# shuaigroup/Renormalizer

Measured on AMD Instinct MI355X. Metric: TDVP-PS sweep site-updates/sec at (Nsite=50, Dbond=256, dphys=2/16), higher is better.
Workload: dtype c128

## Files before the change

include/mpsengine.h:

```cpp
#ifndef MPSENGINE_H
#define MPSENGINE_H

#include <stddef.h>
#include <stdint.h>

#ifdef __cplusplus
extern "C" {
#endif

typedef struct mpse_ctx mpse_ctx;

enum {
  MPSE_OK = 0,
  MPSE_ERR_OOM = 1,
  MPSE_ERR_SHAPE = 2,
  MPSE_ERR_NOCONV = 3,
  MPSE_ERR_HIP = 4,
  MPSE_ERR_ARG = 5
};

enum { MPSE_F64 = 0, MPSE_C128 = 1 };
enum { MPSE_DOMAIN_L = 0, MPSE_DOMAIN_R = 1 };


// ... 56 lines not shown
  int conj_a, conj_b;
  mpse_index m_a, k_a;
  mpse_index k_b, n_b;
  mpse_index m_c, n_c;
  int64_t batch;
  int64_t sb_a, sb_b, sb_c;
  double alpha_re, alpha_im;
  double beta_re, beta_im;
  int skip_zero_tiles;
} mpse_gemm_desc;

int mpse_gemm(mpse_ctx* ctx, const mpse_gemm_desc* desc, const void* A, const void* B, void* C);

int mpse_gemm_path_stats(mpse_ctx* ctx, int64_t* counts, int n);

int mpse_transpose_inner(mpse_ctx* ctx, int dtype, void* out, const void* in,
                         int64_t d0, int64_t d1, int64_t d2, int conj);


typedef struct {
  int64_t Dl_bra, Dl_ket;
  int64_t Dr_bra, Dr_ket;
  int64_t d0, d1;
  int64_t danc;
  int64_t wl, wm, wr;
  int64_t env_unit;
  int64_t danc1;
} mpse_dims;

int mpse_env_update(mpse_ctx* ctx, int dtype, int domain, const mpse_dims* dims,
// ... 159 lines not shown
```

renormalizer_amd/csrc/mpse_cholqr.hip:

```cpp
#include <type_traits>

#include "mpse_device.h"
#include "mpse_internal.h"

typedef double v4d __attribute__((ext_vector_type(4)));

namespace {

struct CqBlk {
  long long ws_off;
  long long part_off;
  long long t_off;
  long long row_off, col_off;
  int mm, nn, P, T;
  int nchunk, rpc;
  int koff, pad;
};

__device__ __forceinline__ v4d mfma(double a, double b, v4d c) {
  return __builtin_amdgcn_mfma_f64_16x16x4f64(a, b, c, 0, 0, 0);
}
__device__ __forceinline__ double readlane_d(double v, int l) {
  const int lo = __builtin_amdgcn_readlane(__double2loint(v), l);
  const int hi = __builtin_amdgcn_readlane(__double2hiint(v), l);
// ... 775 lines not shown
        st2<CPLX>(Vt, (koff + c) * ncol + cols[r], vr, -vi);
      }
    } else {
      const long long u = t - tq;
      const int c = (int)(u % nn), i = (int)(u / nn);
      double vr = 0.0, vi = 0.0;
      if (i <= c) ld2<CPLX>(Rt, (long long)tile_index(i >> 4, c >> 4, B.P) * 256 + (i & 15) * 16 + (c & 15), vr, vi);
      if (!herm)
        st2<CPLX>(Vt, (koff + i) * ncol + cols[c], vr, vi);
      else
        st2<CPLX>(U, rows[c] * K + koff + i, vr, -vi);
    }
  }
}

template <bool CPLX>
int cholqr_run(mpse_ctx* ctx, double* ws, const QrBlk* blks, int nblk, const long long* drows, const long long* dcols,
               int herm, void* U, void* Vt, long long K, long long ncol, bool* ok) {
  MPSE_TRY(qr_words(ctx));
  int* gflag = ctx->qr_optimistic ? ctx->qr_words_dev : nullptr;
  constexpr size_t es = CPLX ? 16 : 8;
  std::vector<CqBlk> cb(nblk);
  long long part_tot = 0, t_tot = 0;
  int max_gram = 1, max_T = 1, max_nrb = 1, max_P = 1;
  long long max_sc = 1;
  long long groups = 0;
  for (int b = 0; b < nblk; ++b) {
    const int P2 = ((blks[b].nn + 15) / 16 + 1) / 2;
    groups += P2 * (P2 + 1) / 2;
  }
  for (int b = 0; b < nblk; ++b) {
    CqBlk& c = cb[b];
    c.ws_off = blks[b].ws_off;
    c.mm = blks[b].mm;
    c.nn = blks[b].nn;
    c.P = (c.nn + 15) / 16;
    c.T = c.P * (c.P + 1) / 2;
    c.row_off = blks[b].row_off;
    c.col_off = blks[b].col_off;
    c.koff = blks[b].prm_off;
    c.pad = 0;
    int want = (int)((8LL * ctx->n_cu + groups - 1) / groups);
    if (want < 1) want = 1;
    if (want > 64) want = 64;
    int rpc = (c.mm + want - 1) / want;
    if (rpc < 32) rpc = 32;
    rpc = (rpc + 3) & ~3;
    c.rpc = rpc;
    c.nchunk = (c.mm + rpc - 1) / rpc;
    c.part_off = part_tot;
    c.t_off = t_tot;
    part_tot += (long long)((c.nchunk + 3) / 4) * c.T * 256;
    t_tot += c.T;
    {
      const int P2 = (c.P + 1) / 2, T2 = P2 * (P2 + 1) / 2;
      max_gram = std::max(max_gram, ((c.nchunk + 3) / 4) * T2);
    }
    max_T = std::max(max_T, c.T);
    max_P = std::max(max_P, c.P);
    max_nrb = std::max(max_nrb, (c.mm + 15) / 16);
    max_sc = std::max<long long>(max_sc, (long long)c.mm * c.nn + (long long)c.nn * c.nn);
  }
  const size_t db = (size_t(nblk) * sizeof(CqBlk) + 15) & ~size_t(15);
  const size_t pb = size_t(part_tot) * es, tb = size_t(t_tot) * 256 * es, ib = size_t(t_tot) * 2 * sizeof(double);
  const size_t sb = ((2 * size_t(nblk) + 1) * sizeof(int) + 15) & ~size_t(15);
  TmpBuf M(ctx);
  MPSE_TRY(M.alloc(db + pb + 6 * tb + ib + sb + 16));
  char* base = static_cast<char*>(M.p);
  MPSE_TRY(stage_h2d(ctx, base, cb.data(), size_t(nblk) * sizeof(CqBlk)));
  const CqBlk* dblk = reinterpret_cast<const CqBlk*>(base);
  double* part = reinterpret_cast<double*>(base + db);
  double* G = reinterpret_cast<double*>(base + db + pb);
  double* Rb[5];
  for (int i = 0; i < 5; ++i) Rb[i] = reinterpret_cast<double*>(base + db + pb + (1 + i) * tb);
  double* tinfo = reinterpret_cast<double*>(base + db + pb + 6 * tb);
  int* status = reinterpret_cast<int*>(base + db + pb + 6 * tb + ib);
  const int* done = status + 1 + nblk;
  double* dstat = reinterpret_cast<double*>(base + db + pb + 6 * tb + ib + sb);
  static const double theta = [] {
    const char* e = getenv("MPSE_CHOLQR_THETA");
    return e ? atof(e) : 1e-12;
  }();
  static const double tau = [] {
    const char* e = getenv("MPSE_CHOLQR_TAU");
    return e ? atof(e) : 0.1;
// ... 45 lines not shown
  static const int min_rows = [] {
    const char* e = getenv("MPSE_CHOLQR_MINROWS");
    return e ? atoi(e) : 256;
  }();
  if (mode == 0 || nblk <= 0) return false;
  int max_mm = 0, max_nn = 0;
  for (int b = 0; b < nblk; ++b) {
    if (blks[b].mm < blks[b].nn || blks[b].k != blks[b].nn || blks[b].nn > 256) return false;
    max_mm = std::max(max_mm, blks[b].mm);
    max_nn = std::max(max_nn, blks[b].nn);
  }
  if (mode >= 2) return true;
  return max_mm >= min_rows && max_nn >= 96;
}

int cholqr_blocks(mpse_ctx* ctx, bool cplx, double* ws, const QrBlk* blks, int nblk, const long long* drows,
                  const long long* dcols, int herm, void* U, void* Vt, long long K, long long ncol, bool* ok) {
  *ok = false;
  if (cplx) return cholqr_run<true>(ctx, ws, blks, nblk, drows, dcols, herm, U, Vt, K, ncol, ok);
  return cholqr_run<false>(ctx, ws, blks, nblk, drows, dcols, herm, U, Vt, K, ncol, ok);
}
```

renormalizer_amd/csrc/mpse_gemm.hip:

```cpp
#include <cstdlib>

#include "mpse_device.h"
#include "mpse_internal.h"
#include "mpse_plans.h"

typedef double v4d __attribute__((ext_vector_type(4)));

static unsigned long long* gemm_trace_ptr(const mpse_ctx* ctx) {
  static const bool f0_only = [] {
    const char* e = getenv("MPSE_GEMM_TRACE_ONLY");
    return e && e[0] == 'f';
  }();
  return (ctx->prof_on && !f0_only) ? ctx->gemm_trace : nullptr;
}

namespace {

struct IdxMap {
  long long s_hi, s_lo;
  int ext, lo;
};

constexpr int GMAX_GRP = 8, GMAX_SEG = 4, GMAX_MIX = 8;
struct GMix {
// ... 865 lines not shown
      dre = dim = 0.0;
#pragma unroll
      for (int w = 0; w < NT / 64; ++w) {
        dre += s_dot[2 * w];
        dim += s_dot[2 * w + 1];
      }
      if (tid == 0) {
        const long long slot = (long long)bs * ntile + (long long)tm * g.tiles_n + tn;
        g.dot_part[2 * slot] = dre;
        g.dot_part[2 * slot + 1] = dim;
      }
    }
  }
}

__device__ __forceinline__ void bitonic_desc(unsigned* key, int tid, int n) {
  for (int size = 2; size <= n; size <<= 1)
    for (int stride = size >> 1; stride > 0; stride >>= 1) {
      if (tid < (n >> 1)) {
        const int lo = 2 * tid - (tid & (stride - 1)), hi = lo + stride;
        const bool desc = (lo & size) == 0;
        const unsigned a = key[lo], b = key[hi];
        if ((a < b) == desc) {
          key[lo] = b;
          key[hi] = a;
        }
      }
      __syncthreads();
    }
}
__device__ __forceinline__ int pow2_at_least(int x) {
  int n = 2;
  while (n < x) n <<= 1;
  return n;
}
__global__ __launch_bounds__(1024) void k_tile_order(const unsigned long long* __restrict__ amask,
                                                       const unsigned long long* __restrict__ bmask, int nkw, int nkt,
                                                       int tiles_m, int tiles_n, int by_die, int* __restrict__ perm,
                                                       const int* __restrict__ skip, const GemmGroups gg,
                                                       unsigned char* __restrict__ flags_out, int flags_pitch,
                                                       int om_M, int om_N) {
  if (skip && *skip) return;
  __shared__ unsigned key[2048], ckey[2048];
  __shared__ int colw[2048];
  __shared__ unsigned char die_of[2048], dead[2048];
  const int ntile = tiles_m * tiles_n, tid = threadIdx.x;
  const bool part = by_die && tiles_n % 8 == 0 && tiles_n <= 2048;
  for (int c = tid; c < 2048; c += 1024) colw[c] = 0;
  __syncthreads();
  for (int i = tid; i < 2048; i += 1024) {
    unsigned cnt = 0;
    dead[i] = 0;
    if (i < ntile) {
      const int tm = i / tiles_n, tn = i - tm * tiles_n;
      if (gg.ngrp > 0) {
        const int grp = tm / gg.tiles_m_grp, tml = tm - grp * gg.tiles_m_grp;
        const GGrp& G = gg.g[grp];
        const bool off = gg.omask && !mpse_plan::out_tile_live(gg.omask, gg.om_pitch, gg.om_d, om_N, om_M, tm, tn);
        dead[i] = off ? 1 : 0;
        for (int q = 0; q < G.nseg; ++q)
          for (int l = 0; l < gg.nkt_seg; ++l) {
            unsigned v = off ? 0 : 1;
            if (G.seg[q].am) v &= G.seg[q].am[(long long)tml * gg.am_pitch + l];
            if (G.seg[q].bm) v &= G.seg[q].bm[(long long)tn * gg.bm_pitch + l];
            cnt += v;
            if (flags_out) flags_out[(long long)i * flags_pitch + q * gg.nkt_seg + l] = (unsigned char)v;
          }
        if (flags_out)
          for (int l = G.nseg * gg.nkt_seg; l < flags_pitch; ++l) flags_out[(long long)i * flags_pitch + l] = 0;
      } else {
        for (int w = 0; w < nkw; ++w) {
          unsigned long long x = 0x0101010101010101ull;
          if (amask) x &= amask[(long long)tm * nkw + w];
          if (bmask) x &= bmask[(long long)tn * nkw + w];
          const int valid = nkt - 8 * w;
          if (valid < 8) x &= (1ull << (8 * valid)) - 1ull;
          cnt += __popcll(x);
        }
      }
      if (part) atomicAdd(&colw[tn], (int)cnt);
    }
    key[i] = cnt;
  }
  __syncthreads();
  if (part) {
    for (int c = tid; c < 2048; c += 1024) ckey[c] = c < tiles_n ? ((unsigned)colw[c] << 11) | (unsigned)(2047 - c) : 0u;
    __syncthreads();
    bitonic_desc(ckey, tid, pow2_at_least(tiles_n));
    for (int r = tid; r < tiles_n; r += 1024) {
      const int c = 2047 - (int)(ckey[r] & 2047u), r16 = r & 15;
      die_of[c] = (unsigned char)(r16 < 8 ? r16 : 15 - r16);
    }
    __syncthreads();
  }
  for (int i = tid; i < 2048; i += 1024) {
    unsigned k = 0;
    if (i < ntile) {
      const unsigned die = part ? die_of[i % tiles_n] : 0u;
      k = (die << 28) | (key[i] << 16) | (unsigned)(0xFFFF - i);
    }
    key[i] = k;
  }
  __syncthreads();
  bitonic_desc(key, tid, pow2_at_least(ntile));
  const int per_die = ntile / 8;
  for (int i = tid; i < ntile; i += 1024) {
    const int s = part ? (7 - (i & 7)) * per_die + (i >> 3) : i;
    const int t = 0xFFFF - (int)(key[s] & 0xFFFFu);
    perm[i] = dead[t] ? ~t : t;
  }
}

template <bool CC>
__global__ __launch_bounds__(256) void k_splitk_reduce(const GemmArgs g, int batch) {
  constexpr int EC = CC ? 2 : 1;
  if (g.skip && *g.skip) return;
  const long long mn = (long long)g.M * g.N;
  const int rows = g.M * batch;
  double dre = 0.0, dim = 0.0;
  for (int row = blockIdx.y; row < rows; row += gridDim.y) {
    const int b = row / g.M;
    const int i = row - b * g.M;
    const double* wrow = g.ws + ((long long)b * g.ksplit * mn + (long long)i * g.N) * EC;
    double* crow = g.C + ((long long)b * g.sbC + idx_off(g.mC, i)) * EC;
    for (int j = blockIdx.x * 256 + threadIdx.x; j < g.N; j += gridDim.x * 256) {
// ... 406 lines not shown
      const OccOperand oa = occ_operand(ka, g.mA, g.kA, g.a_kfast, ma), ob = occ_operand(kb, g.nB, g.kB, g.b_kfast, mb);
      const dim3 og((p.nkt + 3) / 4, oa.tiles > ob.tiles ? oa.tiles : ob.tiles, (unsigned)(2 * d->batch));
      hipLaunchKernelGGL(k_tile_occ, og, dim3(256), 0, ctx->stream, oa, ob, g.K, g.nkw, (int)d->batch, g.skip);
    }
    g.amask = static_cast<const unsigned long long*>(ma.mask);
    g.bmask = static_cast<const unsigned long long*>(mb.mask);
  }

  if (p.order) {
    SolveScope* const keep = sc && sc->keeps_env_masks && ma.stable && mb.stable ? sc : nullptr;
    int* pp = nullptr;
    bool sort = false;
    MPSE_TRY(perm_source(ctx, keep, {g.amask, g.bmask, g.tiles_m, g.tiles_n, p.nkt, nullptr},
                         size_t(g.tiles_m) * g.tiles_n * sizeof(int), PERM, &pp, &sort));
    if (sort)
      hipLaunchKernelGGL(k_tile_order, dim3(1), dim3(1024), 0, ctx->stream, g.amask, g.bmask, g.nkw, p.nkt, g.tiles_m,
                         g.tiles_n, 1, pp, g.skip, GemmGroups(), (unsigned char*)nullptr, 0, 0, 0);
    g.perm = pp;
  }

  count_paths(ctx->gemm_paths, p, d->batch > 1);
  const bool reduce = g.ksplit > 1 && !p.leave_slices;
  launch_gemm(ctx, g, p.nwg, ca, cb, p.fast, p.wide, false, reduce ? dim3((unsigned)p.rgx, (unsigned)p.rgy) : dim3(0),
              (int)d->batch);
  if (prof_this) prof_end(ctx, rec);
  MPSE_HIP(ctx, hipGetLastError());
  return MPSE_OK;
}

int occ_mask_get(mpse_ctx* ctx, SolveScope* sc, const void* ptr, int dtype, mpse_index r, mpse_index k,
                 TmpBuf& tmp, const unsigned char** flags, int* pitch, bool* stable) {
  IdxMap rm, km;
// ... 130 lines not shown
  const bool prof_this = prof_begin(ctx, variant, mnk * ((ca && cb) ? 8.0 : 4.0),
                                    grouped_bytes(d, double(g.M), double(g.N), double(g.K), ca),
                                    &rec);
  g.kt_counter = prof_this && ctx->prof_ktiles ? ctx->prof_ktiles + variant : nullptr;

  TmpBuf PERM(ctx);
  if (p.order) {
    const size_t perm_bytes = (size_t(ntile) * sizeof(int) + 7) & ~size_t(7), flag_pitch = size_t(g.nkw) * 8;
    int* pp = nullptr;
    bool sort = false;
    MPSE_TRY(perm_source(ctx, sc && sc->keeps_env_masks && d.masks_stable ? sc : nullptr,
                         {gg.g[0].seg[0].am, gg.g[0].seg[0].bm, g.tiles_m, g.tiles_n,
                          nkt_max + 1000 * d.ngrp + (out_mask ? 1000000 : 0), nullptr},
                         perm_bytes + size_t(ntile) * flag_pitch, PERM, &pp, &sort));
    if (sort)
      hipLaunchKernelGGL(k_tile_order, dim3(1), dim3(1024), 0, ctx->stream, (const unsigned long long*)nullptr,
                         (const unsigned long long*)nullptr, 0, nkt_max, g.tiles_m, g.tiles_n, d.split2 ? 0 : 1, pp,
                         g.skip, gg, reinterpret_cast<unsigned char*>(pp) + perm_bytes, (int)flag_pitch, g.M, g.N);
    g.perm = pp;
    g.gg.flags = reinterpret_cast<const unsigned long long*>(reinterpret_cast<const char*>(pp) + perm_bytes);
  }

  count_paths(ctx->gemm_paths, d);
  ctx->gemm_paths[mpse_ctx::GP_GROUPED_OUTMASK] += out_mask;
  const bool om_wide = out_mask && d.split2 && ca && !p.wide && g.N % BN == 0;
  gg.dot4 = om_wide ? 1 : 0;
  launch_gemm(ctx, g, p.nwg, ca, cb, true, p.wide || om_wide, true);
  if (prof_this) prof_end(ctx, rec);
  MPSE_HIP(ctx, hipGetLastError());
  return MPSE_OK;
}

extern "C" int mpse_gemm(mpse_ctx* ctx, const mpse_gemm_desc* d, const void* A, const void* B, void* C) {
  if (ctx && d && MPSE_RECORDING(ctx)) {
    const mpse_gemm_desc dc = *d;
    ctx->defer_ops[ctx->defer_recording].push_back([ctx, dc, A, B, C] { return mpse_gemm(ctx, &dc, A, B, C); });
    return MPSE_OK;
  }
  return gemm_impl(ctx, d, A, B, C, d ? (d->skip_zero_tiles & 3) : 0, nullptr, nullptr);
}

extern "C" int mpse_gemm_path_stats(mpse_ctx* ctx, int64_t* counts, int n) {
  if (!ctx || n < 0 || (n > 0 && !counts)) return MPSE_ERR_ARG;
  for (int i = 0; i < n && i < mpse_ctx::GP_COUNT; ++i) counts[i] = ctx->gemm_paths[i];
  return MPSE_OK;
}

int gemm_call(mpse_ctx* ctx, int dta, int dtb, int conja, int conjb, mpse_index ma, mpse_index ka, mpse_index kb,
              mpse_index nb, mpse_index mc, mpse_index nc, int64_t batch, int64_t sba, int64_t sbb, int64_t sbc,
              const void* A, const void* B, void* C, double alpha, double beta, int skip_zero, SolveScope* sc,
              ProductReq* rq) {
  mpse_gemm_desc d;
  d.dtype_a = dta;
  d.dtype_b = dtb;
  d.conj_a = conja;
  d.conj_b = conjb;
  d.m_a = ma;
  d.k_a = ka;
  d.k_b = kb;
// ... 34 lines not shown
```

renormalizer_amd/csrc/mpse_heff0.hip:

```cpp
#include "mpse_device.h"
#include "mpse_internal.h"

typedef double v4d __attribute__((ext_vector_type(4)));

namespace {

__device__ __forceinline__ v4d mfma(double a, double b, v4d c) {
  return __builtin_amdgcn_mfma_f64_16x16x4f64(a, b, c, 0, 0, 0);
}

constexpr int F0_TMAX = 16;
struct F0Term {
  int b, e, x, pad;
  double w;
};
struct F0Info {
  int unit;
  int nt;
  unsigned long long lts;
  unsigned long long frn;
  unsigned long long cts;
  unsigned bpack, epack;
  double w[4];
};
// ... 31 lines not shown
__device__ __forceinline__ void f0_flags(const double2* __restrict__ E, int D, int w, int nt, unsigned char* __restrict__ F,
                                         int rt, int b) {
  __shared__ int s_f[64];
  const int row = threadIdx.x >> 4, col = threadIdx.x & 15;
  if (threadIdx.x < 64) s_f[threadIdx.x] = 0;
  __syncthreads();
  const double2* base = E + ((long long)(16 * rt + row) * w + b) * D;
  for (int ct = 0; ct < nt; ++ct) {
    const double2 v = base[16 * ct + col];
    if (v.x != 0.0 || v.y != 0.0) s_f[ct] = 1;
  }
  __syncthreads();
  if ((int)threadIdx.x < nt) F[((long long)rt * w + b) * nt + threadIdx.x] = s_f[threadIdx.x] ? 1 : 0;
}

__global__ __launch_bounds__(256) void k_f0_prepare(const double2* __restrict__ L, const double2* __restrict__ R,
                                                     double2* __restrict__ rt, unsigned char* __restrict__ FL,
                                                     unsigned char* __restrict__ FR, int Dl, int Dr, int wl, int wr, int ntl,
                                                     int ntr, const int* __restrict__ skip) {
  if (skip && *skip) return;
  int blk = blockIdx.x;
  if (blk < ntl * wl) {
    f0_flags(L, Dl, wl, ntl, FL, blk / wl, blk % wl);
    return;
  }
  blk -= ntl * wl;
  if (blk < ntr * wr) {
    f0_flags(R, Dr, wr, ntr, FR, blk / wr, blk % wr);
    return;
  }
  blk -= ntr * wr;
  f0_transpose(rt, R, Dr, wr, blk, (int)gridDim.x - ntl * wl - ntr * wr);
}

__global__ __launch_bounds__(1024) void k_f0_valid(const unsigned char* __restrict__ FL, const unsigned char* __restrict__ FC,
                                                    const unsigned char* __restrict__ FR, const F0Term* __restrict__ terms,
                                                    const int* __restrict__ nterm, int wl, int wr, int d, int ntl, int ntr,
                                                    int nkc, int fc_pitch, unsigned long long* __restrict__ mask,
                                                    const int* __restrict__ skip) {
  if (skip && *skip) return;
  __shared__ unsigned long long s1[64], s2[64];
  const int nparts = wr * nkc, tid = threadIdx.x;
  if (tid < 64) s1[tid] = s2[tid] = 0;
  __syncthreads();
  for (int t = tid; t < ntl * nparts; t += 1024) {
    const int at = t / nparts, s = t - at * nparts, f = s / nkc, kc = s - f * nkc;
    bool any = false;
// ... 494 lines not shown
  const size_t o_fl = rt_bytes, o_fr = o_fl + fl_bytes, o_tm = o_fr + fr_bytes, o_nt = o_tm + tm_bytes, o_mk = o_nt + nt_bytes;
  const size_t o_od = o_mk + mk_bytes, tot_bytes = o_od + od_bytes;
  static const bool order_on = [] {
    const char* e = getenv("MPSE_F0_ORDER");
    return !(e && e[0] == '0');
  }();
  if (hit) {
    base = static_cast<char*>(fc.buf);
  } else {
    void* p = nullptr;
    if (fc.buf) mpse_free(ctx, fc.buf);
    fc = SolveScope::F0Cache();
    MPSE_TRY(mpse_malloc(ctx, tot_bytes, &p));
    fc.buf = p, fc.L = h->L, fc.R = h->R, fc.W = h->W0, fc.cmask = FC, fc.Dl = Dl, fc.Dr = Dr, fc.w = wr, fc.nsite = h->nsite;
    base = static_cast<char*>(p);
    {
      std::vector<char> up(tm_bytes + nt_bytes, 0);
      memcpy(up.data(), terms.data(), tm_bytes);
      memcpy(up.data() + tm_bytes, nterm.data(), size_t(wr) * sizeof(int));
      MPSE_TRY(stage_h2d(ctx, base + o_tm, up.data(), up.size()));
    }
    const long long nel = (long long)wr * Dr * Dr;
    int nb = (int)((nel + 255) / 256);
    if (nb > 2048) nb = 2048;
    hipLaunchKernelGGL(k_f0_prepare, dim3(ntl * wl + ntr * wr + nb), dim3(256), 0, ctx->stream,
                       static_cast<const double2*>(h->L), static_cast<const double2*>(h->R), reinterpret_cast<double2*>(base),
                       reinterpret_cast<unsigned char*>(base + o_fl), reinterpret_cast<unsigned char*>(base + o_fr), Dl, Dr, wl,
                       wr, ntl, ntr, skip);
    if (order_on)
      hipLaunchKernelGGL(k_f0_plan, dim3(1), dim3(1024), 0, ctx->stream, reinterpret_cast<const unsigned char*>(base + o_fl), FC,
                         reinterpret_cast<const unsigned char*>(base + o_fr), reinterpret_cast<const F0Term*>(base + o_tm),
                         reinterpret_cast<const int*>(base + o_nt), wl, wr, d, ntl, ntr, nkc, fc_pitch,
                         reinterpret_cast<unsigned long long*>(base + o_mk), ctx->n_cu > 0 ? ctx->n_cu : 256,
                         reinterpret_cast<F0Info*>(base + o_od), compact ? 1 : 0, skip);
    else
      hipLaunchKernelGGL(k_f0_valid, dim3(1), dim3(1024), 0, ctx->stream, reinterpret_cast<const unsigned char*>(base + o_fl), FC,
                         reinterpret_cast<const unsigned char*>(base + o_fr), reinterpret_cast<const F0Term*>(base + o_tm),
                         reinterpret_cast<const int*>(base + o_nt), wl, wr, d, ntl, ntr, nkc, fc_pitch,
                         reinterpret_cast<unsigned long long*>(base + o_mk), skip);
  }
  F0Args g{};
  g.L = static_cast<const double*>(h->L);
  g.Rt = reinterpret_cast<const double*>(base);
// ... 44 lines not shown
```

renormalizer_amd/csrc/mpse_internal.h:

```cpp
#pragma once
#include <hip/hip_runtime.h>

#include <cstdarg>
#include <cstdlib>
#include <cstdint>
#include <cstdio>
#include <cstring>
#include <functional>
#include <map>
#include <memory>
#include <mutex>
#include <string>
#include <unordered_map>
#include <vector>

#include "../../include/mpsengine.h"

struct mpse_ctx {
  int device = 0;
  hipStream_t stream = nullptr;
  int n_cu = 0;
  char err[512] = {0};
  char dev_name[128] = {0};

// ... 410 lines not shown
};
struct QrBlk {
  long long ws_off;
  long long q_off;
  int mm, nn, k;
  int prm_off;
  int nq = 0;
  long long row_off = 0, col_off = 0;
};
constexpr int HH_BATCH_MAX_ROWS = 4096;
constexpr unsigned long long GEMM_TRACE_CAP = 1ull << 21;
constexpr int GEMM_TRACE_WORDS = 10;
int hh_qr(mpse_ctx* ctx, bool cplx, double* ws, double* q, HhParam* prm, const QrBlk* blks_host, int nblk, bool form_q,
          const QrBlk* blks_dev = nullptr);
bool cholqr_eligible(const mpse_ctx* ctx, const QrBlk* blks, int nblk);
int cholqr_blocks(mpse_ctx* ctx, bool cplx, double* ws, const QrBlk* blks, int nblk, const long long* drows,
                  const long long* dcols, int herm, void* U, void* Vt, long long K, long long ncol, bool* ok);
int device_zero2(mpse_ctx* ctx, void* a, size_t abytes, void* b, size_t bbytes);
```

renormalizer_amd/csrc/mpse_qr.hip:

```cpp
#include "mpse_cx.h"
#include "mpse_device.h"
#include "mpse_internal.h"

namespace {

template <bool CPLX>
__global__ void k_gather_blocks(double* ws_base, const double* __restrict__ coef, long long ncol,
                                const long long* __restrict__ drows, const long long* __restrict__ dcols,
                                const QrBlk* __restrict__ blks, int herm) {
  const QrBlk B = blks[blockIdx.y];
  double* ws = ws_base + B.ws_off * Cx<CPLX>::E;
  const long long* rows = drows + B.row_off;
  const long long* cols = dcols + B.col_off;
  const int mm = B.mm, nn = B.nn;
  const long long total = (long long)mm * nn;
  const long long stride = (long long)gridDim.x * blockDim.x;
  for (long long t = (long long)blockIdx.x * blockDim.x + threadIdx.x; t < total; t += stride) {
    int r, c;
    if (!herm) {
      c = (int)(t % nn);
      r = (int)(t / nn);
      Cx<CPLX>::st(ws, r + (long long)c * mm, Cx<CPLX>::ld(coef, rows[r] * ncol + cols[c]));
    } else {
      r = (int)(t % mm);
// ... 83 lines not shown
  const int64_t nri = row_off[nblocks], nci = col_off[nblocks];
  int64_t max_el = 0, max_sc = 0;
  for (size_t i = 0; i < blks.size(); ++i) {
    blks[i].row_off = row_off[which[i]];
    blks[i].col_off = col_off[which[i]];
    max_el = std::max<int64_t>(max_el, (int64_t)blks[i].mm * blks[i].nn);
    max_sc = std::max<int64_t>(max_sc, (int64_t)blks[i].mm * blks[i].k + (int64_t)blks[i].k * blks[i].nn);
  }
  double qr_flops = 0.0, qr_bytes = 0.0;
  for (const QrBlk& B : blks) {
    const double m = B.mm, n = B.k;
    qr_flops += (CPLX ? 4.0 : 1.0) * (4.0 * m * n * n - 4.0 * n * n * n / 3.0);
    qr_bytes += double(es) * (2.0 * B.mm * B.nn + double(B.mm) * B.k);
  }
  ProfScope qprof(ctx, 5, qr_flops, qr_bytes);
  const size_t ib = size_t(nri + nci) * sizeof(int64_t), db = blks.size() * sizeof(QrBlk);
  static_assert(sizeof(QrBlk) % 8 == 0, "descriptors follow the 8-byte index lists");
  std::vector<char> host(ib + db);
  memcpy(host.data(), row_idx, size_t(nri) * sizeof(int64_t));
  memcpy(host.data() + size_t(nri) * sizeof(int64_t), col_idx, size_t(nci) * sizeof(int64_t));
  memcpy(host.data() + ib, blks.data(), db);
  TmpBuf IDX(ctx), WS(ctx), Q(ctx), PRM(ctx);
  MPSE_TRY(IDX.alloc(ib + db));
  MPSE_TRY(WS.alloc(size_t(ws_tot) * es));
  MPSE_TRY(stage_h2d(ctx, IDX.p, host.data(), ib + db));
  const long long* drows = static_cast<const long long*>(IDX.p);
  const long long* dcols = drows + nri;
  const QrBlk* dblk = reinterpret_cast<const QrBlk*>(static_cast<const char*>(IDX.p) + ib);
  double* ws = static_cast<double*>(WS.p);
  ++ctx->qr_calls;
  hipLaunchKernelGGL((k_gather_blocks<CPLX>), dim3(ew_blocks(max_el), (unsigned)blks.size()), dim3(256), 0, ctx->stream, ws,
                     (const double*)coef, (long long)ncol, drows, dcols, dblk, herm);
  if (!hh_only && cholqr_eligible(ctx, blks.data(), (int)blks.size())) {
    bool ok = false;
    MPSE_TRY(cholqr_blocks(ctx, CPLX, ws, blks.data(), (int)blks.size(), drows, dcols, herm, U, Vt, (long long)K,
                           (long long)ncol, &ok));
    ++ctx->qr_chol_calls;
    if (ok) {
      qprof.end();
      return MPSE_OK;
    }
    ++ctx->qr_chol_fallbacks;
    hipLaunchKernelGGL((k_gather_blocks<CPLX>), dim3(ew_blocks(max_el), (unsigned)blks.size()), dim3(256), 0, ctx->stream,
                       ws, (const double*)coef, (long long)ncol, drows, dcols, dblk, herm);
  }
  MPSE_TRY(Q.alloc(size_t(q_tot) * es));
  MPSE_TRY(PRM.alloc(size_t(ktot + 1) * sizeof(HhParam)));
  double* q = static_cast<double*>(Q.p);
  HhParam* prm = static_cast<HhParam*>(PRM.p);
  MPSE_TRY(hh_qr(ctx, CPLX, ws, q, prm, blks.data(), (int)blks.size(), true, dblk));
  hipLaunchKernelGGL((k_scatter_blocks<CPLX>), dim3(ew_blocks(max_sc), (unsigned)blks.size()), dim3(256), 0, ctx->stream,
// ... 169 lines not shown
```

renormalizer_amd/engine.py:

```python
import collections
import ctypes as C
import math
import os
import threading

import numpy as np

_HERE = os.path.dirname(os.path.abspath(__file__))
LIB_PATH = os.environ.get("RENO_MPSENGINE") or os.path.join(_HERE, "csrc", "libmpsengine.so")

F64, C128 = 0, 1
MPSE_OK, MPSE_ERR_OOM, MPSE_ERR_SHAPE, MPSE_ERR_NOCONV, MPSE_ERR_HIP, MPSE_ERR_ARG = 0, 1, 2, 3, 4, 5
DOMAIN_L, DOMAIN_R = 0, 1

STATUS = {0: "OK", 1: "OOM", 2: "SHAPE", 3: "NOCONV", 4: "HIP", 5: "ARG"}


PcgResult = collections.namedtuple("PcgResult", "status iters relres lvalue")


class EngineError(RuntimeError):
    pass


# ... 94 lines not shown
    "mpse_mul_real": [C.c_void_p, C.c_int, C.c_void_p, C.c_void_p, C.c_int64],
    "mpse_davidson_precond": [C.c_void_p, C.c_int, C.c_void_p, C.c_void_p, C.c_void_p, C.c_void_p, C.c_int64,
                              C.c_double, C.c_double],
    "mpse_real_part": [C.c_void_p, C.c_void_p, C.c_void_p, C.c_int64],
    "mpse_dotc": [C.c_void_p, C.c_int, C.c_void_p, C.c_void_p, C.c_int64, _dblp],
    "mpse_nrm2": [C.c_void_p, C.c_int, C.c_void_p, C.c_int64, _dblp],
    "mpse_scaled_rms": [C.c_void_p, C.c_int, C.c_void_p, C.c_void_p, C.c_void_p, C.c_int64, C.c_double, C.c_double, _dblp],
    "mpse_expm_centre_mask": [C.c_void_p, C.c_void_p, C.c_int64],
    "mpse_defer_begin": [C.c_void_p, C.c_int],
    "mpse_defer_end": [C.c_void_p],
    "mpse_defer_arm": [C.c_void_p, C.c_int],
    "mpse_defer_run": [C.c_void_p, C.c_int],
    "mpse_defer_discard": [C.c_void_p],
    "mpse_gemm": [C.c_void_p, C.POINTER(mpse_gemm_desc), C.c_void_p, C.c_void_p, C.c_void_p],
    "mpse_gemm_path_stats": [C.c_void_p, _i64p, C.c_int],
    "mpse_transpose_inner": [C.c_void_p, C.c_int, C.c_void_p, C.c_void_p, C.c_int64, C.c_int64, C.c_int64, C.c_int],
    "mpse_env_update": [C.c_void_p, C.c_int, C.c_int, C.POINTER(mpse_dims), C.c_void_p, C.c_int, C.c_void_p,
                        C.c_void_p, C.c_int, C.c_void_p, C.c_int, C.c_void_p],
    "mpse_heff_apply": [C.c_void_p, C.c_int, C.POINTER(mpse_heff), C.c_void_p, C.c_void_p],
    "mpse_heff_apply2": [C.c_void_p, C.c_int, C.POINTER(mpse_heff), C.c_void_p, C.c_void_p],
    "mpse_env_update_multi": [C.c_void_p, C.c_int, C.c_int, C.POINTER(mpse_dims), C.c_int, _i64p, _i64p, C.c_void_p,
                              C.c_int, C.c_void_p, C.c_void_p, C.c_int, C.POINTER(C.c_void_p), C.c_int, C.c_void_p],
    "mpse_env_unit_channel": [C.c_void_p, C.c_int, C.c_void_p, C.c_int64, C.c_int64, C.c_double, _i64p],
    "mpse_expm_lanczos": [C.c_void_p, C.c_int, C.POINTER(mpse_heff), C.c_double, C.c_double, C.c_void_p, C.c_void_p,
                          C.c_double, C.c_double, C.c_int, C.POINTER(C.c_int)],
    "mpse_expm_lanczos_batch": [C.c_void_p, C.c_int, C.c_int, C.POINTER(mpse_heff), C.c_double, C.c_double,
                                C.POINTER(C.c_void_p), C.POINTER(C.c_void_p), C.c_double, C.c_double, C.c_int,
                                C.POINTER(C.c_int)],
    "mpse_expm_lanczos_batch_stats": [C.c_void_p, _i64p, _i64p],
    "mpse_expm_lanczos_path_stats": [C.c_void_p, _i64p, C.c_int],
# ... 874 lines not shown
```

Baseline: 612.9.

## Merge small host uploads into launches and speed up tile-order kernel

Cholesky-QR block descriptors are now computed on the host and packed into the same staging upload as the QR index lists, so cholqr skips its own separate upload. The F0 term table is passed as a kernel argument and written by an extra block of the prepare kernel, which removes another host-to-device staging copy. The tile-order kernel gains a variant that uses wavefront barriers instead of block barriers for small bitonic strides, plus 8-byte-word mask ANDs with popcount and a more memory-parallel output-mask liveness check. A debug entry point for testing tile ordering is also added. The intent is to cut per-call launch and synchronisation overhead, at the cost of more complex code paths selected by environment variables.

Result: no change. 607.0 (-1.0%).

```diff
diff --git a/include/mpsengine.h b/include/mpsengine.h
--- a/include/mpsengine.h
+++ b/include/mpsengine.h
@@ -94,6 +94,11 @@
 
 int mpse_gemm_path_stats(mpse_ctx* ctx, int64_t* counts, int n);
 
+int mpse_debug_tile_order(mpse_ctx* ctx, int tiles_m, int tiles_n, int nkt, int by_die, const unsigned char* amask,
+                          const unsigned char* bmask, int ngrp, int nseg, const unsigned char* omask, int om_pitch,
+                          int om_rows, int om_d, int om_M, int om_N, int flags_pitch, int32_t* perm,
+                          unsigned char* flags_out);
+
 int mpse_transpose_inner(mpse_ctx* ctx, int dtype, void* out, const void* in,
                          int64_t d0, int64_t d1, int64_t d2, int conj);
 
diff --git a/renormalizer_amd/csrc/mpse_cholqr.hip b/renormalizer_amd/csrc/mpse_cholqr.hip
--- a/renormalizer_amd/csrc/mpse_cholqr.hip
+++ b/renormalizer_amd/csrc/mpse_cholqr.hip
@@ -813,23 +813,21 @@
   }
 }
 
-template <bool CPLX>
-int cholqr_run(mpse_ctx* ctx, double* ws, const QrBlk* blks, int nblk, const long long* drows, const long long* dcols,
-               int herm, void* U, void* Vt, long long K, long long ncol, bool* ok) {
-  MPSE_TRY(qr_words(ctx));
-  int* gflag = ctx->qr_optimistic ? ctx->qr_words_dev : nullptr;
-  constexpr size_t es = CPLX ? 16 : 8;
-  std::vector<CqBlk> cb(nblk);
-  long long part_tot = 0, t_tot = 0;
+struct CqPlan {
+  std::vector<CqBlk> cb;
+  long long part_tot = 0, t_tot = 0, max_sc = 1;
   int max_gram = 1, max_T = 1, max_nrb = 1, max_P = 1;
-  long long max_sc = 1;
+};
+CqPlan cq_plan(const mpse_ctx* ctx, const QrBlk* blks, int nblk) {
+  CqPlan p;
+  p.cb.resize(nblk);
   long long groups = 0;
   for (int b = 0; b < nblk; ++b) {
     const int P2 = ((blks[b].nn + 15) / 16 + 1) / 2;
     groups += P2 * (P2 + 1) / 2;
   }
   for (int b = 0; b < nblk; ++b) {
-    CqBlk& c = cb[b];
+    CqBlk& c = p.cb[b];
     c.ws_off = blks[b].ws_off;
     c.mm = blks[b].mm;
     c.nn = blks[b].nn;
@@ -847,27 +845,40 @@
     rpc = (rpc + 3) & ~3;
     c.rpc = rpc;
     c.nchunk = (c.mm + rpc - 1) / rpc;
-    c.part_off = part_tot;
-    c.t_off = t_tot;
-    part_tot += (long long)((c.nchunk + 3) / 4) * c.T * 256;
-    t_tot += c.T;
+    c.part_off = p.part_tot;
+    c.t_off = p.t_tot;
+    p.part_tot += (long long)((c.nchunk + 3) / 4) * c.T * 256;
+    p.t_tot += c.T;
     {
       const int P2 = (c.P + 1) / 2, T2 = P2 * (P2 + 1) / 2;
-      max_gram = std::max(max_gram, ((c.nchunk + 3) / 4) * T2);
-    }
-    max_T = std::max(max_T, c.T);
-    max_P = std::max(max_P, c.P);
-    max_nrb = std::max(max_nrb, (c.mm + 15) / 16);
-    max_sc = std::max<long long>(max_sc, (long long)c.mm * c.nn + (long long)c.nn * c.nn);
-  }
+      p.max_gram = std::max(p.max_gram, ((c.nchunk + 3) / 4) * T2);
+    }
+    p.max_T = std::max(p.max_T, c.T);
+    p.max_P = std::max(p.max_P, c.P);
+    p.max_nrb = std::max(p.max_nrb, (c.mm + 15) / 16);
+    p.max_sc = std::max<long long>(p.max_sc, (long long)c.mm * c.nn + (long long)c.nn * c.nn);
+  }
+  return p;
+}
+
+template <bool CPLX>
+int cholqr_run(mpse_ctx* ctx, double* ws, const QrBlk* blks, int nblk, const long long* drows, const long long* dcols,
+               int herm, void* U, void* Vt, long long K, long long ncol, bool* ok, const void* desc_dev) {
+  MPSE_TRY(qr_words(ctx));
+  int* gflag = ctx->qr_optimistic ? ctx->qr_words_dev : nullptr;
+  constexpr size_t es = CPLX ? 16 : 8;
+  const CqPlan pl = cq_plan(ctx, blks, nblk);
+  const std::vector<CqBlk>& cb = pl.cb;
+  const long long part_tot = pl.part_tot, t_tot = pl.t_tot, max_sc = pl.max_sc;
+  const int max_gram = pl.max_gram, max_T = pl.max_T, max_nrb = pl.max_nrb, max_P = pl.max_P;
   const size_t db = (size_t(nblk) * sizeof(CqBlk) + 15) & ~size_t(15);
   const size_t pb = size_t(part_tot) * es, tb = size_t(t_tot) * 256 * es, ib = size_t(t_tot) * 2 * sizeof(double);
   const size_t sb = ((2 * size_t(nblk) + 1) * sizeof(int) + 15) & ~size_t(15);
   TmpBuf M(ctx);
   MPSE_TRY(M.alloc(db + pb + 6 * tb + ib + sb + 16));
   char* base = static_cast<char*>(M.p);
-  MPSE_TRY(stage_h2d(ctx, base, cb.data(), size_t(nblk) * sizeof(CqBlk)));
-  const CqBlk* dblk = reinterpret_cast<const CqBlk*>(base);
+  if (!desc_dev) MPSE_TRY(stage_h2d(ctx, base, cb.data(), size_t(nblk) * sizeof(CqBlk)));
+  const CqBlk* dblk = desc_dev ? static_cast<const CqBlk*>(desc_dev) : reinterpret_cast<const CqBlk*>(base);
   double* part = reinterpret_cast<double*>(base + db);
   double* G = reinterpret_cast<double*>(base + db + pb);
   double* Rb[5];
@@ -943,9 +954,16 @@
   return max_mm >= min_rows && max_nn >= 96;
 }
 
+size_t cholqr_desc_bytes(int nblk) { return size_t(nblk) * sizeof(CqBlk); }
+void cholqr_desc_fill(const mpse_ctx* ctx, const QrBlk* blks, int nblk, void* out) {
+  const CqPlan pl = cq_plan(ctx, blks, nblk);
+  memcpy(out, pl.cb.data(), cholqr_desc_bytes(nblk));
+}
+
 int cholqr_blocks(mpse_ctx* ctx, bool cplx, double* ws, const QrBlk* blks, int nblk, const long long* drows,
-                  const long long* dcols, int herm, void* U, void* Vt, long long K, long long ncol, bool* ok) {
+                  const long long* dcols, int herm, void* U, void* Vt, long long K, long long ncol, bool* ok,
+                  const void* desc_dev) {
   *ok = false;
-  if (cplx) return cholqr_run<true>(ctx, ws, blks, nblk, drows, dcols, herm, U, Vt, K, ncol, ok);
-  return cholqr_run<false>(ctx, ws, blks, nblk, drows, dcols, herm, U, Vt, K, ncol, ok);
-}
+  if (cplx) return cholqr_run<true>(ctx, ws, blks, nblk, drows, dcols, herm, U, Vt, K, ncol, ok, desc_dev);
+  return cholqr_run<false>(ctx, ws, blks, nblk, drows, dcols, herm, U, Vt, K, ncol, ok, desc_dev);
+}
diff --git a/renormalizer_amd/csrc/mpse_gemm.hip b/renormalizer_amd/csrc/mpse_gemm.hip
--- a/renormalizer_amd/csrc/mpse_gemm.hip
+++ b/renormalizer_amd/csrc/mpse_gemm.hip
@@ -903,6 +903,7 @@
   }
 }
 
+template <bool WAVE>
 __device__ __forceinline__ void bitonic_desc(unsigned* key, int tid, int n) {
   for (int size = 2; size <= n; size <<= 1)
     for (int stride = size >> 1; stride > 0; stride >>= 1) {
@@ -915,7 +916,13 @@
           key[hi] = a;
         }
       }
-      __syncthreads();
+      if (!WAVE || stride >= 128 || (stride == 1 && (size >= 128 || size == n))) {
+        __syncthreads();
+      } else {
+        __builtin_amdgcn_fence(__ATOMIC_RELEASE, "wavefront");
+        __builtin_amdgcn_wave_barrier();
+        __builtin_amdgcn_fence(__ATOMIC_ACQUIRE, "wavefront");
+      }
     }
 }
 __device__ __forceinline__ int pow2_at_least(int x) {
@@ -923,6 +930,27 @@
   while (n < x) n <<= 1;
   return n;
 }
+constexpr int TO_MLP = 8;
+__device__ __forceinline__ bool out_tile_live_mlp(const unsigned char* __restrict__ mask, int pitch, int d, int Dr, int M,
+                                                  int tm, int tn) {
+  const int r1 = 64 * tm + 64 < M ? 64 * tm + 64 : M, l0 = 64 * tn, l1 = 64 * tn + 63 < Dr - 1 ? 64 * tn + 63 : Dr - 1;
+  unsigned any = 0;
+  for (int r0 = 64 * tm; r0 < r1; r0 += TO_MLP) {
+    unsigned char v[2 * TO_MLP];
+#pragma unroll
+    for (int u = 0; u < TO_MLP; ++u) {
+      const int r = r0 + u < r1 ? r0 + u : r1 - 1;
+      const int a = r / d, sg = r - a * d;
+      const int c0 = (sg * Dr + l0) >> 6, c1 = (sg * Dr + l1) >> 6;
+      v[2 * u] = c0 <= c1 ? mask[(long long)c0 * pitch + (a >> 4)] : 0;
+      v[2 * u + 1] = c0 <= c1 ? mask[(long long)c1 * pitch + (a >> 4)] : 0;
+    }
+#pragma unroll
+    for (int u = 0; u < 2 * TO_MLP; ++u) any |= v[u];
+  }
+  return any != 0;
+}
+template <bool WAVE>
 __global__ __launch_bounds__(1024) void k_tile_order(const unsigned long long* __restrict__ amask,
                                                        const unsigned long long* __restrict__ bmask, int nkw, int nkt,
                                                        int tiles_m, int tiles_n, int by_die, int* __restrict__ perm,
@@ -945,18 +973,70 @@
       if (gg.ngrp > 0) {
         const int grp = tm / gg.tiles_m_grp, tml = tm - grp * gg.tiles_m_grp;
         const GGrp& G = gg.g[grp];
-        const bool off = gg.omask && !mpse_plan::out_tile_live(gg.omask, gg.om_pitch, gg.om_d, om_N, om_M, tm, tn);
+        bool off;
+        if constexpr (WAVE)
+          off = gg.omask && !out_tile_live_mlp(gg.omask, gg.om_pitch, gg.om_d, om_N, om_M, tm, tn);
+        else
+          off = gg.omask && !mpse_plan::out_tile_live(gg.omask, gg.om_pitch, gg.om_d, om_N, om_M, tm, tn);
         dead[i] = off ? 1 : 0;
-        for (int q = 0; q < G.nseg; ++q)
+        for (int q = 0; q < G.nseg; ++q) {
+          const unsigned char* const am = G.seg[q].am ? G.seg[q].am + (long long)tml * gg.am_pitch : nullptr;
+          const unsigned char* const bm = G.seg[q].bm ? G.seg[q].bm + (long long)tn * gg.bm_pitch : nullptr;
+          unsigned char* const fo = flags_out ? flags_out + (long long)i * flags_pitch + q * gg.nkt_seg : nullptr;
+          if (WAVE && gg.nkt_seg % 8 == 0 && ((reinterpret_cast<uintptr_t>(am) | reinterpret_cast<uintptr_t>(bm) |
+                                               reinterpret_cast<uintptr_t>(fo)) & 7) == 0) {
+            const int nw = gg.nkt_seg / 8;
+            const unsigned long long* const aw = reinterpret_cast<const unsigned long long*>(am);
+            const unsigned long long* const bw = reinterpret_cast<const unsigned long long*>(bm);
+            unsigned long long* const fw = reinterpret_cast<unsigned long long*>(fo);
+            for (int w0 = 0; w0 < nw; w0 += TO_MLP) {
+              unsigned long long x[TO_MLP];
+#pragma unroll
+              for (int u = 0; u < TO_MLP; ++u) {
+                x[u] = off ? 0ull : 0x0101010101010101ull;
+                if (aw && !off && w0 + u < nw) x[u] &= aw[w0 + u];
+              }
+#pragma unroll
+              for (int u = 0; u < TO_MLP; ++u)
+                if (bw && !off && w0 + u < nw) x[u] &= bw[w0 + u];
+#pragma unroll
+              for (int u = 0; u < TO_MLP; ++u)
+                if (w0 + u < nw) {
+                  cnt += __popcll(x[u]);
+                  if (fw) fw[w0 + u] = x[u];
+                }
+            }
+            continue;
+          }
           for (int l = 0; l < gg.nkt_seg; ++l) {
             unsigned v = off ? 0 : 1;
-            if (G.seg[q].am) v &= G.seg[q].am[(long long)tml * gg.am_pitch + l];
-            if (G.seg[q].bm) v &= G.seg[q].bm[(long long)tn * gg.bm_pitch + l];
+            if (am) v &= am[l];
+            if (bm) v &= bm[l];
             cnt += v;
-            if (flags_out) flags_out[(long long)i * flags_pitch + q * gg.nkt_seg + l] = (unsigned char)v;
+            if (fo) fo[l] = (unsigned char)v;
           }
+        }
         if (flags_out)
           for (int l = G.nseg * gg.nkt_seg; l < flags_pitch; ++l) flags_out[(long long)i * flags_pitch + l] = 0;
+      } else if constexpr (WAVE) {
+        for (int w0 = 0; w0 < nkw; w0 += TO_MLP) {
+          unsigned long long x[TO_MLP];
+#pragma unroll
+          for (int u = 0; u < TO_MLP; ++u) {
+            x[u] = 0x0101010101010101ull;
+            if (amask && w0 + u < nkw) x[u] &= amask[(long long)tm * nkw + w0 + u];
+          }
+#pragma unroll
+          for (int u = 0; u < TO_MLP; ++u)
+            if (bmask && w0 + u < nkw) x[u] &= bmask[(long long)tn * nkw + w0 + u];
+#pragma unroll
+          for (int u = 0; u < TO_MLP; ++u)
+            if (w0 + u < nkw) {
+              const int valid = nkt - 8 * (w0 + u);
+              if (valid < 8) x[u] &= (1ull << (8 * valid)) - 1ull;
+              cnt += __popcll(x[u]);
+            }
+        }
       } else {
         for (int w = 0; w < nkw; ++w) {
           unsigned long long x = 0x0101010101010101ull;
@@ -975,7 +1055,7 @@
   if (part) {
     for (int c = tid; c < 2048; c += 1024) ckey[c] = c < tiles_n ? ((unsigned)colw[c] << 11) | (unsigned)(2047 - c) : 0u;
     __syncthreads();
-    bitonic_desc(ckey, tid, pow2_at_least(tiles_n));
+    bitonic_desc<WAVE>(ckey, tid, pow2_at_least(tiles_n));
     for (int r = tid; r < tiles_n; r += 1024) {
       const int c = 2047 - (int)(ckey[r] & 2047u), r16 = r & 15;
       die_of[c] = (unsigned char)(r16 < 8 ? r16 : 15 - r16);
@@ -991,13 +1071,26 @@
     key[i] = k;
   }
   __syncthreads();
-  bitonic_desc(key, tid, pow2_at_least(ntile));
+  bitonic_desc<WAVE>(key, tid, pow2_at_least(ntile));
   const int per_die = ntile / 8;
   for (int i = tid; i < ntile; i += 1024) {
     const int s = part ? (7 - (i & 7)) * per_die + (i >> 3) : i;
     const int t = 0xFFFF - (int)(key[s] & 0xFFFFu);
     perm[i] = dead[t] ? ~t : t;
   }
+}
+bool tile_order_wave() {
+  static const bool on = [] {
+    const char* e = getenv("MPSE_TILE_ORDER");
+    return !(e && e[0] == '0');
+  }();
+  return on;
+}
+void launch_tile_order(hipStream_t stream, bool wave, const unsigned long long* amask, const unsigned long long* bmask,
+                       int nkw, int nkt, int tiles_m, int tiles_n, int by_die, int* perm, const int* skip,
+                       const GemmGroups& gg, unsigned char* flags_out, int flags_pitch, int om_M, int om_N) {
+  hipLaunchKernelGGL(wave ? k_tile_order<true> : k_tile_order<false>, dim3(1), dim3(1024), 0, stream, amask, bmask, nkw,
+                     nkt, tiles_m, tiles_n, by_die, perm, skip, gg, flags_out, flags_pitch, om_M, om_N);
 }
 
 template <bool CC>
@@ -1434,8 +1527,8 @@
     MPSE_TRY(perm_source(ctx, keep, {g.amask, g.bmask, g.tiles_m, g.tiles_n, p.nkt, nullptr},
                          size_t(g.tiles_m) * g.tiles_n * sizeof(int), PERM, &pp, &sort));
     if (sort)
-      hipLaunchKernelGGL(k_tile_order, dim3(1), dim3(1024), 0, ctx->stream, g.amask, g.bmask, g.nkw, p.nkt, g.tiles_m,
-                         g.tiles_n, 1, pp, g.skip, GemmGroups(), (unsigned char*)nullptr, 0, 0, 0);
+      launch_tile_order(ctx->stream, tile_order_wave(), g.amask, g.bmask, g.nkw, p.nkt, g.tiles_m, g.tiles_n, 1, pp,
+                        g.skip, GemmGroups(), nullptr, 0, 0, 0);
     g.perm = pp;
   }
 
@@ -1596,9 +1689,9 @@
                           nkt_max + 1000 * d.ngrp + (out_mask ? 1000000 : 0), nullptr},
                          perm_bytes + size_t(ntile) * flag_pitch, PERM, &pp, &sort));
     if (sort)
-      hipLaunchKernelGGL(k_tile_order, dim3(1), dim3(1024), 0, ctx->stream, (const unsigned long long*)nullptr,
-                         (const unsigned long long*)nullptr, 0, nkt_max, g.tiles_m, g.tiles_n, d.split2 ? 0 : 1, pp,
-                         g.skip, gg, reinterpret_cast<unsigned char*>(pp) + perm_bytes, (int)flag_pitch, g.M, g.N);
+      launch_tile_order(ctx->stream, tile_order_wave(), nullptr, nullptr, 0, nkt_max, g.tiles_m, g.tiles_n,
+                        d.split2 ? 0 : 1, pp, g.skip, gg, reinterpret_cast<unsigned char*>(pp) + perm_bytes,
+                        (int)flag_pitch, g.M, g.N);
     g.perm = pp;
     g.gg.flags = reinterpret_cast<const unsigned long long*>(reinterpret_cast<const char*>(pp) + perm_bytes);
   }
@@ -1625,6 +1718,68 @@
 extern "C" int mpse_gemm_path_stats(mpse_ctx* ctx, int64_t* counts, int n) {
   if (!ctx || n < 0 || (n > 0 && !counts)) return MPSE_ERR_ARG;
   for (int i = 0; i < n && i < mpse_ctx::GP_COUNT; ++i) counts[i] = ctx->gemm_paths[i];
+  return MPSE_OK;
+}
+
+extern "C" int mpse_debug_tile_order(mpse_ctx* ctx, int tiles_m, int tiles_n, int nkt, int by_die,
+                                     const unsigned char* amask, const unsigned char* bmask, int ngrp, int nseg,
+                                     const unsigned char* omask, int om_pitch, int om_rows, int om_d, int om_M, int om_N,
+                                     int flags_pitch, int32_t* perm, unsigned char* flags_out) {
+  if (!ctx || !perm || tiles_m < 1 || tiles_n < 1 || nkt < 1 || nkt > 512 || ngrp < 0 || ngrp > GMAX_GRP) return MPSE_ERR_ARG;
+  MPSE_BIND(ctx);
+  const long long ntile = (long long)tiles_m * tiles_n;
+  if (ntile > 2048) return mpse_fail(ctx, MPSE_ERR_SHAPE, "mpse_debug_tile_order: more than 2048 tiles");
+  const bool grouped = ngrp > 0;
+  if (grouped && (nseg < 1 || nseg > GMAX_SEG || tiles_m % ngrp || !flags_out || flags_pitch < nseg * nkt ||
+                  (omask && (ngrp != 1 || om_pitch < 1 || om_rows < 1 || om_d < 1))))
+    return MPSE_ERR_ARG;
+  if (!grouped && (omask || flags_out)) return MPSE_ERR_ARG;
+  if (omask && (om_M < 1 || om_N < 1 || (long long)om_rows * 64 < (long long)om_d * om_N ||
+                (long long)om_pitch * 16 * om_d < om_M))
+    return MPSE_ERR_ARG;
+  const int nkw = (nkt + 7) / 8, tmg = grouped ? tiles_m / ngrp : tiles_m;
+  const size_t a_rows = grouped ? size_t(ngrp) * nseg * tmg : size_t(tiles_m);
+  const size_t b_rows = grouped ? size_t(ngrp) * nseg * tiles_n : size_t(tiles_n);
+  const size_t row = grouped ? size_t(nkt) : size_t(nkw) * 8;
+  const auto up8 = [](size_t x) { return (x + 7) & ~size_t(7); };
+  const size_t a_bytes = amask ? up8(a_rows * row) : 0, b_bytes = bmask ? up8(b_rows * row) : 0;
+  const size_t o_bytes = omask ? up8(size_t(om_rows) * om_pitch) : 0;
+  const size_t p_bytes = up8(size_t(ntile) * sizeof(int)), f_bytes = flags_out ? up8(size_t(ntile) * flags_pitch) : 0;
+  TmpBuf buf(ctx);
+  MPSE_TRY(buf.alloc(a_bytes + b_bytes + o_bytes + 2 * (p_bytes + f_bytes)));
+  unsigned char* const da = buf.as<unsigned char>();
+  unsigned char* const db = da + a_bytes;
+  unsigned char* const dom = db + b_bytes;
+  unsigned char* const dout = dom + o_bytes;
+  if (amask) MPSE_HIP(ctx, hipMemcpyAsync(da, amask, a_rows * row, hipMemcpyHostToDevice, ctx->stream));
+  if (bmask) MPSE_HIP(ctx, hipMemcpyAsync(db, bmask, b_rows * row, hipMemcpyHostToDevice, ctx->stream));
+  if (omask) MPSE_HIP(ctx, hipMemcpyAsync(dom, omask, size_t(om_rows) * om_pitch, hipMemcpyHostToDevice, ctx->stream));
+  MPSE_HIP(ctx, hipMemsetAsync(dout, 0xEE, 2 * (p_bytes + f_bytes), ctx->stream));
+  GemmGroups gg{};
+  if (grouped) {
+    gg.ngrp = ngrp, gg.tiles_m_grp = tmg, gg.nkt_seg = nkt, gg.am_pitch = nkt, gg.bm_pitch = nkt;
+    for (int g = 0; g < ngrp; ++g) {
+      gg.g[g].nseg = nseg;
+      for (int q = 0; q < nseg; ++q) {
+        gg.g[g].seg[q].am = amask ? da + (size_t(g) * nseg + q) * tmg * nkt : nullptr;
+        gg.g[g].seg[q].bm = bmask ? db + (size_t(g) * nseg + q) * tiles_n * nkt : nullptr;
+      }
+    }
+    if (omask) gg.omask = dom, gg.om_pitch = om_pitch, gg.om_d = om_d;
+  }
+  for (int v = 0; v < 2; ++v) {
+    unsigned char* const o = dout + size_t(v) * (p_bytes + f_bytes);
+    launch_tile_order(ctx->stream, v == 1, grouped ? nullptr : reinterpret_cast<const unsigned long long*>(amask ? da : nullptr),
+                      grouped ? nullptr : reinterpret_cast<const unsigned long long*>(bmask ? db : nullptr),
+                      grouped ? 0 : nkw, nkt, tiles_m, tiles_n, by_die, reinterpret_cast<int*>(o), nullptr, gg,
+                      flags_out ? o + p_bytes : nullptr, flags_pitch, om_M, om_N);
+    MPSE_HIP(ctx, hipGetLastError());
+    MPSE_HIP(ctx, hipMemcpyAsync(perm + size_t(v) * ntile, o, size_t(ntile) * sizeof(int), hipMemcpyDeviceToHost, ctx->stream));
+    if (flags_out)
+      MPSE_HIP(ctx, hipMemcpyAsync(flags_out + size_t(v) * ntile * flags_pitch, o + p_bytes, size_t(ntile) * flags_pitch,
+                                   hipMemcpyDeviceToHost, ctx->stream));
+  }
+  MPSE_HIP(ctx, hipStreamSynchronize(ctx->stream));
   return MPSE_OK;
 }
 
diff --git a/renormalizer_amd/csrc/mpse_heff0.hip b/renormalizer_amd/csrc/mpse_heff0.hip
--- a/renormalizer_amd/csrc/mpse_heff0.hip
+++ b/renormalizer_amd/csrc/mpse_heff0.hip
@@ -69,12 +69,20 @@
   if ((int)threadIdx.x < nt) F[((long long)rt * w + b) * nt + threadIdx.x] = s_f[threadIdx.x] ? 1 : 0;
 }
 
+struct F0Table {
+  unsigned long long w[256];
+};
 __global__ __launch_bounds__(256) void k_f0_prepare(const double2* __restrict__ L, const double2* __restrict__ R,
                                                      double2* __restrict__ rt, unsigned char* __restrict__ FL,
                                                      unsigned char* __restrict__ FR, int Dl, int Dr, int wl, int wr, int ntl,
-                                                     int ntr, const int* __restrict__ skip) {
+                                                     int ntr, const int* __restrict__ skip, unsigned long long* __restrict__ tab,
+                                                     int tab_words, const F0Table table) {
   if (skip && *skip) return;
   int blk = blockIdx.x;
+  if (tab_words > 0 && blk == (int)gridDim.x - 1) {
+    if ((int)threadIdx.x < tab_words) tab[threadIdx.x] = table.w[threadIdx.x];
+    return;
+  }
   if (blk < ntl * wl) {
     f0_flags(L, Dl, wl, ntl, FL, blk / wl, blk % wl);
     return;
@@ -85,7 +93,7 @@
     return;
   }
   blk -= ntr * wr;
-  f0_transpose(rt, R, Dr, wr, blk, (int)gridDim.x - ntl * wl - ntr * wr);
+  f0_transpose(rt, R, Dr, wr, blk, (int)gridDim.x - ntl * wl - ntr * wr - (tab_words > 0 ? 1 : 0));
 }
 
 __global__ __launch_bounds__(1024) void k_f0_valid(const unsigned char* __restrict__ FL, const unsigned char* __restrict__ FC,
@@ -610,19 +618,30 @@
     MPSE_TRY(mpse_malloc(ctx, tot_bytes, &p));
     fc.buf = p, fc.L = h->L, fc.R = h->R, fc.W = h->W0, fc.cmask = FC, fc.Dl = Dl, fc.Dr = Dr, fc.w = wr, fc.nsite = h->nsite;
     base = static_cast<char*>(p);
+    static const bool by_arg = [] {
+      const char* e = getenv("MPSE_UPLOAD_MERGE");
+      return !(e && e[0] == '0');
+    }();
+    F0Table table{};
+    const size_t up_bytes = tm_bytes + nt_bytes;
+    const bool tab_arg = by_arg && up_bytes <= sizeof(F0Table);
     {
-      std::vector<char> up(tm_bytes + nt_bytes, 0);
+      std::vector<char> up(tab_arg ? sizeof(F0Table) : up_bytes, 0);
       memcpy(up.data(), terms.data(), tm_bytes);
       memcpy(up.data() + tm_bytes, nterm.data(), size_t(wr) * sizeof(int));
-      MPSE_TRY(stage_h2d(ctx, base + o_tm, up.data(), up.size()));
+      if (tab_arg)
+        memcpy(&table, up.data(), sizeof(F0Table));
+      else
+        MPSE_TRY(stage_h2d(ctx, base + o_tm, up.data(), up.size()));
     }
     const long long nel = (long long)wr * Dr * Dr;
     int nb = (int)((nel + 255) / 256);
     if (nb > 2048) nb = 2048;
-    hipLaunchKernelGGL(k_f0_prepare, dim3(ntl * wl + ntr * wr + nb), dim3(256), 0, ctx->stream,
+    hipLaunchKernelGGL(k_f0_prepare, dim3(ntl * wl + ntr * wr + nb + (tab_arg ? 1 : 0)), dim3(256), 0, ctx->stream,
                        static_cast<const double2*>(h->L), static_cast<const double2*>(h->R), reinterpret_cast<double2*>(base),
                        reinterpret_cast<unsigned char*>(base + o_fl), reinterpret_cast<unsigned char*>(base + o_fr), Dl, Dr, wl,
-                       wr, ntl, ntr, skip);
+                       wr, ntl, ntr, skip, reinterpret_cast<unsigned long long*>(base + o_tm),
+                       tab_arg ? (int)(up_bytes / 8) : 0, table);
     if (order_on)
       hipLaunchKernelGGL(k_f0_plan, dim3(1), dim3(1024), 0, ctx->stream, reinterpret_cast<const unsigned char*>(base + o_fl), FC,
                          reinterpret_cast<const unsigned char*>(base + o_fr), reinterpret_cast<const F0Term*>(base + o_tm),
diff --git a/renormalizer_amd/csrc/mpse_internal.h b/renormalizer_amd/csrc/mpse_internal.h
--- a/renormalizer_amd/csrc/mpse_internal.h
+++ b/renormalizer_amd/csrc/mpse_internal.h
@@ -448,6 +448,9 @@
 int hh_qr(mpse_ctx* ctx, bool cplx, double* ws, double* q, HhParam* prm, const QrBlk* blks_host, int nblk, bool form_q,
           const QrBlk* blks_dev = nullptr);
 bool cholqr_eligible(const mpse_ctx* ctx, const QrBlk* blks, int nblk);
+size_t cholqr_desc_bytes(int nblk);
+void cholqr_desc_fill(const mpse_ctx* ctx, const QrBlk* blks, int nblk, void* out);
 int cholqr_blocks(mpse_ctx* ctx, bool cplx, double* ws, const QrBlk* blks, int nblk, const long long* drows,
-                  const long long* dcols, int herm, void* U, void* Vt, long long K, long long ncol, bool* ok);
+                  const long long* dcols, int herm, void* U, void* Vt, long long K, long long ncol, bool* ok,
+                  const void* desc_dev = nullptr);
 int device_zero2(mpse_ctx* ctx, void* a, size_t abytes, void* b, size_t bbytes);
diff --git a/renormalizer_amd/csrc/mpse_qr.hip b/renormalizer_amd/csrc/mpse_qr.hip
--- a/renormalizer_amd/csrc/mpse_qr.hip
+++ b/renormalizer_amd/csrc/mpse_qr.hip
@@ -121,16 +121,23 @@
     qr_bytes += double(es) * (2.0 * B.mm * B.nn + double(B.mm) * B.k);
   }
   ProfScope qprof(ctx, 5, qr_flops, qr_bytes);
+  static const bool merge_on = [] {
+    const char* e = getenv("MPSE_UPLOAD_MERGE");
+    return !(e && e[0] == '0');
+  }();
+  const bool chol = !hh_only && cholqr_eligible(ctx, blks.data(), (int)blks.size());
   const size_t ib = size_t(nri + nci) * sizeof(int64_t), db = blks.size() * sizeof(QrBlk);
+  const size_t cb = chol && merge_on ? cholqr_desc_bytes((int)blks.size()) : 0;
   static_assert(sizeof(QrBlk) % 8 == 0, "descriptors follow the 8-byte index lists");
-  std::vector<char> host(ib + db);
+  std::vector<char> host(ib + db + cb);
   memcpy(host.data(), row_idx, size_t(nri) * sizeof(int64_t));
   memcpy(host.data() + size_t(nri) * sizeof(int64_t), col_idx, size_t(nci) * sizeof(int64_t));
   memcpy(host.data() + ib, blks.data(), db);
+  if (cb) cholqr_desc_fill(ctx, blks.data(), (int)blks.size(), host.data() + ib + db);
   TmpBuf IDX(ctx), WS(ctx), Q(ctx), PRM(ctx);
-  MPSE_TRY(IDX.alloc(ib + db));
+  MPSE_TRY(IDX.alloc(ib + db + cb));
   MPSE_TRY(WS.alloc(size_t(ws_tot) * es));
-  MPSE_TRY(stage_h2d(ctx, IDX.p, host.data(), ib + db));
+  MPSE_TRY(stage_h2d(ctx, IDX.p, host.data(), ib + db + cb));
   const long long* drows = static_cast<const long long*>(IDX.p);
   const long long* dcols = drows + nri;
   const QrBlk* dblk = reinterpret_cast<const QrBlk*>(static_cast<const char*>(IDX.p) + ib);
@@ -138,10 +145,10 @@
   ++ctx->qr_calls;
   hipLaunchKernelGGL((k_gather_blocks<CPLX>), dim3(ew_blocks(max_el), (unsigned)blks.size()), dim3(256), 0, ctx->stream, ws,
                      (const double*)coef, (long long)ncol, drows, dcols, dblk, herm);
-  if (!hh_only && cholqr_eligible(ctx, blks.data(), (int)blks.size())) {
+  if (chol) {
     bool ok = false;
     MPSE_TRY(cholqr_blocks(ctx, CPLX, ws, blks.data(), (int)blks.size(), drows, dcols, herm, U, Vt, (long long)K,
-                           (long long)ncol, &ok));
+                           (long long)ncol, &ok, cb ? static_cast<const char*>(IDX.p) + ib + db : nullptr));
     ++ctx->qr_chol_calls;
     if (ok) {
       qprof.end();
diff --git a/renormalizer_amd/engine.py b/renormalizer_amd/engine.py
--- a/renormalizer_amd/engine.py
+++ b/renormalizer_amd/engine.py
@@ -132,6 +132,8 @@
     "mpse_defer_discard": [C.c_void_p],
     "mpse_gemm": [C.c_void_p, C.POINTER(mpse_gemm_desc), C.c_void_p, C.c_void_p, C.c_void_p],
     "mpse_gemm_path_stats": [C.c_void_p, _i64p, C.c_int],
+    "mpse_debug_tile_order": [C.c_void_p] + [C.c_int] * 4 + [C.c_void_p] * 2 + [C.c_int] * 2 + [C.c_void_p] +
+                             [C.c_int] * 6 + [C.c_void_p] * 2,
     "mpse_transpose_inner": [C.c_void_p, C.c_int, C.c_void_p, C.c_void_p, C.c_int64, C.c_int64, C.c_int64, C.c_int],
     "mpse_env_update": [C.c_void_p, C.c_int, C.c_int, C.POINTER(mpse_dims), C.c_void_p, C.c_int, C.c_void_p,
                         C.c_void_p, C.c_int, C.c_void_p, C.c_int, C.c_void_p],
```
